# imjaegyun/super_resolution

Measured on AMD Instinct MI355X. Metric: SR output megapixels/sec, HAT-S x4, 1280x720 LR in, higher is better.
Workload: dtype bf16; 1 GPU; HAT-S x4, one 3x720x1280 LR frame per GPU, full-frame forward; upscale=4, parallelism=dp1

## Files before the change

super_resolution_amd/csrc/hat_mlp.hip:

```cpp
#include <type_traits>

#include "hat_common.h"

namespace {

struct LdsBases { unsigned b0, b1, b2; };
constexpr unsigned LB_STEP = 61440;
__device__ __forceinline__ LdsBases lds_bases(const char* lane_base) {
    typedef __attribute__((address_space(3))) char lds_char;
    LdsBases r;
    r.b0 = (unsigned)(uintptr_t)(lds_char*)lane_base;
    r.b1 = r.b0 + LB_STEP;
    r.b2 = r.b0 + 2 * LB_STEP;
    asm volatile("" : "+v"(r.b0), "+v"(r.b1), "+v"(r.b2));
    return r;
}
template <typename V> __device__ __forceinline__ V lds_at(const LdsBases& lb, unsigned off) {
    const unsigned base = off < LB_STEP ? lb.b0 : (off < 2 * LB_STEP ? lb.b1 : lb.b2);
    const unsigned rel = off < LB_STEP ? off : (off < 2 * LB_STEP ? off - LB_STEP : off - 2 * LB_STEP);
    return *(__attribute__((address_space(3))) const V*)(uintptr_t)(base + rel);
}

constexpr int ML_C = 144, ML_HID = 288, ML_NT1 = ML_HID / 16, ML_NT2 = ML_C / 16, ML_KK = ML_HID / 32;
constexpr int ML_W1F = ML_NT1 * 4 * 1024;
constexpr int ML_W1H = ML_NT1 * 512;
constexpr int ML_NREG = 4;
constexpr int ML_W2F = (ML_NT2 * ML_KK - ML_NREG) * 1024;
constexpr int ML_OFF_W1H = ML_W1F, ML_OFF_W2 = ML_W1F + ML_W1H, ML_OFF_B1 = ML_OFF_W2 + ML_W2F, ML_OFF_B2 = ML_OFF_B1 + ML_HID * 4;
constexpr int ML_LDS = ML_OFF_B2 + ML_C * 4;
constexpr int ML_WAVES = 8, ML_NTHR = ML_WAVES * 64;

template <bool OUTF32, bool R16 = false>
__global__ __launch_bounds__(ML_NTHR) void ocab_mlp_kernel(const HatMlpDesc d, long npix, long tiles) {
    using M = MT<bf16_t>;
    typedef bf16_t T;
    typedef M::frag_t frag_t;
    extern __shared__ __attribute__((aligned(16))) char smem[];
    const int tid = threadIdx.x, lane = tid & 63, g = lane >> 4, c16 = lane & 15;
    const int wave = tid >> 6;
    {
        const char* w1 = reinterpret_cast<const char*>(d.w1f);
        for (int i = tid; i < (ML_W1F + ML_W1H) / 16; i += ML_NTHR)
            *reinterpret_cast<u32x4*>(smem + (size_t)i * 16) = *reinterpret_cast<const u32x4*>(w1 + (size_t)i * 16);
        const char* w2 = reinterpret_cast<const char*>(d.w2f);
        for (int i = tid; i < ML_W2F / 16; i += ML_NTHR)
            *reinterpret_cast<u32x4*>(smem + ML_OFF_W2 + (size_t)i * 16) = *reinterpret_cast<const u32x4*>(w2 + (size_t)i * 16);
        float* b1 = reinterpret_cast<float*>(smem + ML_OFF_B1);
        for (int i = tid; i < ML_HID; i += ML_NTHR) b1[i] = d.b1[i];
        float* b2 = reinterpret_cast<float*>(smem + ML_OFF_B2);
        for (int i = tid; i < ML_C; i += ML_NTHR) b2[i] = d.b2[i];
    }
    frag_t w2r[ML_NREG];
#pragma unroll
    for (int i = 0; i < ML_NREG; ++i)
        w2r[i] = M::load(reinterpret_cast<const T*>(d.w2f) + (size_t)(ML_NT2 * ML_KK - ML_NREG + i) * 512 + lane * 8);
    __syncthreads();

    const T* xg = reinterpret_cast<const T*>(d.x);
    const float* b1l = reinterpret_cast<const float*>(smem + ML_OFF_B1);
    const float* b2l = reinterpret_cast<const float*>(smem + ML_OFF_B2);
    typedef short s16x4 __attribute__((ext_vector_type(4)));
    struct XB { frag_t f[4]; s16x4 h; };
    auto load_x = [&](long tile, XB& xb) {
        long p = tile * 16 + c16;
        p = p < npix ? p : npix - 1;
        const T* row = xg + p * d.ldx;
#pragma unroll
        for (int ks = 0; ks < 4; ++ks) xb.f[ks] = M::load(row + ks * 32 + 8 * g);
        xb.h = *reinterpret_cast<const s16x4*>(row + 128 + 4 * g);
    };
    using r1_t = std::conditional_t<R16, h4raw, f32x4>;
    auto load_r = [&](long tile, r1_t (&r)[ML_NT2]) {
        long p = tile * 16 + c16;
        p = p < npix ? p : npix - 1;
#pragma unroll
        for (int nt = 0; nt < ML_NT2; ++nt) {
            if constexpr (R16) r[nt] = load_h4raw(reinterpret_cast<const _Float16*>(d.r1) + p * d.ldr1 + nt * 16 + 4 * g);
            else r[nt] = *reinterpret_cast<const f32x4*>(d.r1 + p * d.ldr1 + nt * 16 + 4 * g);
        }
    };

    const long stride = (long)gridDim.x * ML_WAVES;
    long tile = (long)blockIdx.x * ML_WAVES + wave;
    XB xcur, xnxt;
    r1_t r1v[ML_NT2];
    load_x(tile, xcur);
    load_x(tile + stride, xnxt);
    load_r(tile, r1v);
    for (; tile < tiles; tile += stride) {
        const long p = tile * 16 + c16;
        const long pc = p < npix ? p : npix - 1;
        int wofs = lane * 16;
        asm volatile("" : "+v"(wofs));
        const char* wl = smem + wofs;
        const char* wl8 = smem + ML_OFF_W1H + (wofs >> 1);
        const LdsBases lb = lds_bases(wl), lb8 = lds_bases(smem + (wofs >> 1));
        frag_t pf[ML_KK];
        {
            struct W1 { s16x4 h; f32x4 b; frag_t f[4]; };
            W1 ws[2];
            auto rd1 = [&](int nt, W1& w) {
                w.h = lds_at<s16x4>(lb8, ML_OFF_W1H + nt * 512);
                w.b = *reinterpret_cast<const f32x4*>(b1l + nt * 16 + 4 * g);
#pragma unroll
                for (int ks = 0; ks < 4; ++ks) w.f[ks] = lds_at<frag_t>(lb, (nt * 4 + ks) * 1024);
            };
            rd1(0, ws[0]);
            f32x4 a[2];
#pragma unroll
            for (int nt = 0; nt < ML_NT1; ++nt) {
                if (nt + 1 < ML_NT1) rd1(nt + 1, ws[(nt + 1) & 1]);
                const W1& w = ws[nt & 1];
                const f32x4 tail = __builtin_amdgcn_mfma_f32_16x16x16bf16_1k(w.h, xcur.h, w.b, 0, 0, 0);
                f32x4 ai = f32x4{0.f, 0.f, 0.f, 0.f};
#pragma unroll
                for (int ks = 0; ks < 4; ++ks) ai = M::mma(w.f[ks], xcur.f[ks], ai);
                a[nt & 1] = ai + tail;
                if (nt & 1) {
#pragma unroll
                    for (int j = 0; j < 4; ++j) {
                        pf[nt >> 1][j] = (bf16_t)gelu_act<T>(a[0][j]);
                        pf[nt >> 1][4 + j] = (bf16_t)gelu_act<T>(a[1][j]);
                    }
                }
                __builtin_amdgcn_sched_barrier(0);
            }
        }
        f32x4 acc[ML_NT2];
        {
            constexpr int NF = ML_NT2 * ML_KK - ML_NREG, AD = 3;
            frag_t ring[AD + 1];
            auto rd2 = [&](int f) { ring[f % (AD + 1)] = lds_at<frag_t>(lb, ML_OFF_W2 + f * 1024); };
#pragma unroll
            for (int f = 0; f < AD; ++f) rd2(f);
#pragma unroll
            for (int nt = 0; nt < ML_NT2; ++nt) {
                if constexpr (R16) acc[nt] = *reinterpret_cast<const f32x4*>(b2l + nt * 16 + 4 * g) + h4raw_to_f32(r1v[nt]);
                else acc[nt] = *reinterpret_cast<const f32x4*>(b2l + nt * 16 + 4 * g) + r1v[nt];
#pragma unroll
                for (int kk = 0; kk < ML_KK; ++kk) {
                    const int f = nt * ML_KK + kk;
                    if (f + AD < NF) rd2(f + AD);
                    if (f < NF)
                        acc[nt] = M::mma(ring[f % (AD + 1)], pf[kk], acc[nt]);
                    else
                        acc[nt] = M::mma(w2r[f - NF], pf[kk], acc[nt]);
                    __builtin_amdgcn_sched_barrier(0);
                }
            }
        }
        xcur = xnxt;
        if constexpr (OUTF32) {
            float* o = reinterpret_cast<float*>(d.out) + pc * d.ldo;
#pragma unroll
            for (int nt = 0; nt < ML_NT2; ++nt) *reinterpret_cast<f32x4*>(o + nt * 16 + 4 * g) = acc[nt];
        } else {
            bf16_t* o = reinterpret_cast<bf16_t*>(d.out) + pc * d.ldo;
#pragma unroll
            for (int nt = 0; nt + 1 < ML_NT2; nt += 2) store_pair_bf16(o, nt * 16, g, acc[nt], acc[nt + 1]);
            Vec4<T>::store(o + (ML_NT2 - 1) * 16 + 4 * g, acc[ML_NT2 - 1]);
        }
        load_x(tile + 2 * stride, xnxt);
        load_r(tile + stride, r1v);
    }
}

constexpr int QK_NT = 27, QK_N = QK_NT * 16;
constexpr int QK_WF = QK_NT * 4 * 1024, QK_WH = QK_NT * 512, QK_OFF_B = QK_WF + QK_WH, QK_LDS = QK_OFF_B + QK_N * 4;

__global__ __launch_bounds__(ML_NTHR) void ocab_qkv_kernel(const HatMlpDesc d, long npix, long tiles) {
    using M = MT<bf16_t>;
    typedef bf16_t T;
    typedef M::frag_t frag_t;
    typedef short s16x4 __attribute__((ext_vector_type(4)));
    extern __shared__ __attribute__((aligned(16))) char smem[];
    const int tid = threadIdx.x, lane = tid & 63, g = lane >> 4, c16 = lane & 15;
    const int wave = tid >> 6;
    {
        const char* w1 = reinterpret_cast<const char*>(d.w1f);
        for (int i = tid; i < (QK_WF + QK_WH) / 16; i += ML_NTHR)
            *reinterpret_cast<u32x4*>(smem + (size_t)i * 16) = *reinterpret_cast<const u32x4*>(w1 + (size_t)i * 16);
        float* bl = reinterpret_cast<float*>(smem + QK_OFF_B);
        for (int i = tid; i < QK_N; i += ML_NTHR) bl[i] = d.b1[i];
    }
    __syncthreads();
    const T* xg = reinterpret_cast<const T*>(d.x);
    const float* bl = reinterpret_cast<const float*>(smem + QK_OFF_B);
    struct XB { frag_t f[4]; s16x4 h; };
    auto load_x = [&](long tile, XB& xb) {
        long p = tile * 16 + c16;
        p = p < npix ? p : npix - 1;
        const T* row = xg + p * d.ldx;
#pragma unroll
        for (int ks = 0; ks < 4; ++ks) xb.f[ks] = M::load(row + ks * 32 + 8 * g);
        xb.h = *reinterpret_cast<const s16x4*>(row + 128 + 4 * g);
    };
// ... 31 lines not shown
#pragma unroll
            for (int ks = 0; ks < 4; ++ks) ai = M::mma(w.f[ks], xcur.f[ks], ai);
            a[nt & 1] = ai + tail;
            if (nt & 1) store_pair_bf16(o, (nt - 1) * 16, g, a[0], a[1]);
            else if (nt == QK_NT - 1) last = a[0];
            __builtin_amdgcn_sched_barrier(0);
        }
        Vec4<T>::store(o + (QK_NT - 1) * 16 + 4 * g, last);
        xcur = xnxt;
        load_x(tile + 2 * stride, xnxt);
    }
}

}

extern "C" int hat_ocab_qkv(const HatMlpDesc* dp, void* stream) {
    if (!dp) return HAT_EINVAL;
    const HatMlpDesc& d = *dp;
    if (!d.x || !d.w1f || !d.b1 || !d.out || d.B < 1 || d.H < 1 || d.W < 1) return HAT_EINVAL;
    if (d.C != ML_C || d.hidden != QK_N || d.dtype != HAT_BF16) return HAT_EUNSUPPORTED;
    if (d.ldx < ML_C || d.ldx % 8 || d.ldo < QK_N || d.ldo % 8 || reinterpret_cast<uintptr_t>(d.out) % 16) return HAT_EINVAL;
    const long npix = (long)d.B * d.H * d.W, tiles = (npix + 15) / 16;
    int gx = 256;
    if ((long)gx * ML_WAVES > tiles) gx = (int)((tiles + ML_WAVES - 1) / ML_WAVES);
    hipError_t e = hipFuncSetAttribute(reinterpret_cast<const void*>(ocab_qkv_kernel), hipFuncAttributeMaxDynamicSharedMemorySize, QK_LDS);
    if (e != hipSuccess) return (int)e;
    HAT_LAUNCH(ocab_qkv_kernel, dim3(gx), dim3(ML_NTHR), QK_LDS, reinterpret_cast<hipStream_t>(stream), d, npix, tiles);
    return hat_check_launch();
}

extern "C" int hat_ocab_mlp(const HatMlpDesc* dp, void* stream) {
    if (!dp) return HAT_EINVAL;
    const HatMlpDesc& d = *dp;
    if (!d.x || !d.w1f || !d.b1 || !d.w2f || !d.b2 || !d.r1 || !d.out) return HAT_EINVAL;
    if (d.B < 1 || d.H < 1 || d.W < 1) return HAT_EINVAL;
    if (d.C != ML_C || d.hidden != ML_HID || d.dtype != HAT_BF16) return HAT_EUNSUPPORTED;
    if (d.ldx < ML_C || d.ldx % 8 || d.ldr1 < ML_C || d.ldr1 % 4 || d.ldo < ML_C) return HAT_EINVAL;
    if ((d.out_f32 & ~3) != 0 || d.out_f32 == 3) return HAT_EINVAL;
    const bool out_f32 = (d.out_f32 & 1) != 0, r16 = (d.out_f32 & 2) != 0;
    if (r16 && reinterpret_cast<uintptr_t>(d.r1) % 8) return HAT_EINVAL;
    if (out_f32 ? d.ldo % 4 : (d.ldo % 8 || reinterpret_cast<uintptr_t>(d.out) % 16)) return HAT_EINVAL;
    const long npix = (long)d.B * d.H * d.W, tiles = (npix + 15) / 16;
    int gx = 256;
    if ((long)gx * ML_WAVES > tiles) gx = (int)((tiles + ML_WAVES - 1) / ML_WAVES);
    hipStream_t s = reinterpret_cast<hipStream_t>(stream);
    void (*kern)(const HatMlpDesc, long, long) = out_f32 ? ocab_mlp_kernel<true> : r16 ? ocab_mlp_kernel<false, true> : ocab_mlp_kernel<false>;
    hipError_t e = hipFuncSetAttribute(reinterpret_cast<const void*>(kern), hipFuncAttributeMaxDynamicSharedMemorySize, ML_LDS);
    if (e != hipSuccess) return (int)e;
    HAT_LAUNCH(kern, dim3(gx), dim3(ML_NTHR), ML_LDS, s, d, npix, tiles);
    return hat_check_launch();
}
```

super_resolution_amd/engine.py:

```python
from __future__ import annotations

import contextlib
import dataclasses
import math
import os
import warnings
from typing import Dict, Optional

import torch

from . import ops
from .engine_base import EngineBase
from .frame_boundary import FrameBoundary
from .ops import (ACT_GELU, ACT_LRELU, ACT_NONE, O_NCHW_F32, O_NHWC_F32, O_NHWC_T, O_PIXSHUF_T, X_NCHW_F32_MEAN, X_NHWC_F32, X_NHWC_T)
from .packing import _ESC

RGB_MEAN = (0.4488, 0.4371, 0.4040)


def _r8(x: int) -> int:
    return (x + 7) // 8 * 8


def _r4(x: int) -> int:
# ... 36 lines not shown
        return cls(t16_guard=(get("t16_guard") or "defer"), **kw)


class _T16Guard:

    def __init__(self, dev):
        self.slot = torch.zeros(1, dtype=torch.int32, device=dev)
        self.host = torch.zeros(1, dtype=torch.int32).pin_memory()
        self.event = torch.cuda.Event()
        self.pending = 0

    def word(self) -> int:
        return int(self.host[0]) & 0xFFFFFFFF


class _Packed:

    def __getitem__(self, key):
        try:
            return getattr(self, key)
        except AttributeError:
            raise KeyError(key) from None


class _Hab(_Packed):
    fold = ffn = ffn3 = fc1 = fc2 = bias256 = None
    tail = "aggr"
    next_ln = None
    out16 = False


class _Ocab(_Packed):
    qkvf = mlpf = esc = fh0 = fh2 = None


class _Naf(_Packed):

    def __init__(self, c, head, blocks, tail):
        self.c, self.head, self.blocks, self.tail = c, head, blocks, tail


class _Group(_Packed):
    to_conv = ocab16 = out16 = False
    conv_ln = None

    def __init__(self, heads, habs, ocab, conv):
        self.heads, self.habs, self.ocab, self.conv = heads, habs, ocab, conv


class _Fwd:

    def __init__(self, eng, w, B, H, W, band, one_stream):
        self.B, self.H, self.W, self.N = B, H, W, H * W
        self.C, self.dt, self.ldc = eng.C, eng.dtype, _r8(eng.C)
        self.geo = dict(B=B, H=H, W=W, dtype=eng.dtype)
        self.w, self.band, self.one_stream = w, band, one_stream
        self.t = self.gin = w["tA"]
        self.have_n = self.have_n16 = False
        self.nblk = ops.layernorm_blocks()

    def ln(self, src, dst, gb, out_f32=False, gap_c=0):
        ops.layernorm(src, dst, gb[0], gb[1], B=self.B, npix=self.N, C_=self.C, ldy=(self.C if out_f32 else self.ldc),
                      out_f32=out_f32, dtype=self.dt, gap=(self.w["gap"] if gap_c else None), gap_c=gap_c)

    def pooled(self, src, ld, C_, dst, off=0, r0=None, r1=None, c0=0, c1=None):
        bd, w = self.band, self.w
# ... 162 lines not shown
            hb.ffn3 = ops.pack_ffn3(*fw, *hb.n2, dev)
        if (hb.fold is None and C == 180 and fp16_ok and ops.tail3_supported(C, hid2 // 2, dt) and hb.esc.pdim == 16
                and hb.esc.aggr.frag and not opt.no_hab_tail):
            f3 = ops.pack_ffn3(*fw, *hb.n2, dev)
            if ops.hab_tail_supported(f3, hb.esc.aggr, w2raw.shape[1], dt):
                hb.ffn3, hb.tail180_ok = f3, True
                hb.bias256 = torch.zeros(256, **f32)
                hb.bias256[:C] = vec(hb.esc.aggr_keys[1])
        return hb

    def _pack_ocab(self, sd, p, heads):
        cfg, dt, dev, C = self.cfg, self.dtype, self.dev, self.C
        vec = lambda k: sd[k].detach().to(dtype=torch.float32, device=dev).contiguous()
        ws, wse = self.ws, self.wse
        M = ws + wse - 1
        shift = (ws - wse + 1 - (ws - 1)) * (M + 1)
        rot = (torch.arange(M * M) + shift) % (M * M)
        d = C // heads
        qscale = cfg.get("qk_scale") or d ** -0.5
        qlog2 = (ops.ocab_attention_log2_supported(C, heads, ws, wse, dt) and not (self.focus or self.topk < 1.0)
                 and not self.opt.no_attn_log2 and d % 2 == 0 and _r8(C) == C)
        if qlog2:
            qscale = qscale * ops.LOG2E
        table = sd[p + ".relative_position_bias_table"].detach().to(torch.float32).cpu()
        oc = _Ocab()
        oc.n1 = (vec(p + ".norm1.weight"), vec(p + ".norm1.bias"))
        oc.n2 = (vec(p + ".norm2.weight"), vec(p + ".norm2.bias"))
        oc.q = self._lin(sd, p + ".q_proj.weight", p + ".q_proj.bias", scale=qscale)
        oc.kv = self._lin(sd, p + ".kv_proj.weight", p + ".kv_proj.bias")
        oc.proj = self._lin(sd, p + ".proj.weight", p + ".proj.bias")
        oc.mlp0 = self._lin(sd, p + ".mlp.0.weight", p + ".mlp.0.bias")
        oc.mlp2 = self._lin(sd, p + ".mlp.2.weight", p + ".mlp.2.bias")
        if ops.ocab_mlp_supported(C, sd[p + ".mlp.0.weight"].shape[0], dt) and _r8(C) == C and not self.opt.no_ocab_mlp:
            oc.mlpf = ops.pack_ocab_mlp(sd[p + ".mlp.0.weight"], sd[p + ".mlp.0.bias"], sd[p + ".mlp.2.weight"], sd[p + ".mlp.2.bias"], dev)
        oc.bias_rot = table[rot].t().contiguous().to(dev)
        oc.qlog2 = qlog2
        if C == 144 and dt == ops.HAT_BF16 and not cfg.get("ocab_esc_enable", False) and not self.opt.no_ocab_qkv:
            oc.qkvf = ops.pack_ocab_qkv(sd[p + ".q_proj.weight"], sd.get(p + ".q_proj.bias"), sd[p + ".kv_proj.weight"],
                                        sd.get(p + ".kv_proj.bias"), qscale, dev)
        if cfg.get("ocab_esc_enable", False):
            oc.esc = self._esc(sd, p + ".esc_core", p + ".esc_plk", cfg["ocab_esc_pdim"], cfg["ocab_esc_kernel"])
        if self.focus:
            oc.fh0 = ops.pack_conv_weight(sd[p + ".focus_head.0.weight"], sd[p + ".focus_head.0.bias"], dt, dev)
            oc.fh2 = ops.pack_conv_weight(sd[p + ".focus_head.2.weight"], sd[p + ".focus_head.2.bias"], dt, dev)
        return oc

    def _pack_ps(self, sd, key, r):
        w = sd[key + ".weight"]
        o = w.shape[0]
        cps = o // (r * r)
        n = torch.arange(o)
        perm = (n % cps) * (r * r) + n // cps
        return ops.pack_conv_weight(w, sd[key + ".bias"], self.dtype, self.dev, out_perm=perm)

    def _resolve(self):
        layers, dt, C = self.layers, self.dtype, self.C
        escs = [hb.esc for G in layers for hb in G.habs] + [G.ocab.esc for G in layers if G.ocab.esc is not None]
        wide = any(e.npad > 16 for e in escs)
        for gi, G in enumerate(layers):
            oc = G.ocab
            for i, hb in enumerate(G.habs):
                nh = G.habs[i + 1] if i + 1 < len(G.habs) else None
                hb.next_ln = (nh.n1, nh.esc.pdim) if nh is not None else (oc.n1, oc.esc.pdim if oc.esc is not None else 0)
                if hb.fold is not None:
                    hb.tail = "fused144" if hb.tail144_ok and not wide else "aggr_cab"
                else:
                    hb.tail = "fused180" if hb.tail180_ok and hb.next_ln[1] <= 16 else "aggr"
            G.to_conv = bool(G.conv is not None and dt == ops.HAT_BF16 and _r8(C) == C and oc.mlp2.frag and not self.opt.no_bf16_conv_in)
            cv = G.conv
            if cv is not None and dt == ops.HAT_BF16 and not self.opt.no_conv_ln and cv.n_slices == 1 and cv.nout == cv.nt * 16:
                if gi + 1 < len(layers):
                    nhs = layers[gi + 1].habs
                    nxt, gap_c = (nhs[0].n1, nhs[0].esc.pdim) if nhs else (None, 0)
                else:
                    nxt, gap_c = (self.norm, 0) if self.conv_after_body is not None else (None, 0)
                G.conv_ln = (nxt, gap_c) if nxt is not None and gap_c in (0, 4, 8, 12, 16) else None
        self._plan_t16()
        self.u8_fused = self.conv_last_sweep is not None and self.conv_last_sweep[2] == 3
        hab0 = layers[0].habs[0] if layers and layers[0].habs else None
        self._hab0 = hab0
        self._yw = max([16] + [e.npad for e in escs])
        self._kpad = max([hab0.esc.kpad if hab0 else 0] + [G.ocab.esc.kpad for G in layers if G.ocab.esc is not None])

    def _plan_t16(self):
        layers = self.layers
        for G in layers:
            G.ocab16 = G.out16 = False
            for hb in G.habs:
                hb.out16 = False
        if not self.t16:
            return
        tail16 = lambda hb: hb.tail == "fused144" and hb.ffn3.C == 144
        conv16 = lambda G: bool(G.conv is not None and not G.conv.frag and G.conv.ksize > 1 and G.conv.nt == 9
                                and G.conv.n_slices == 1 and G.conv.nout == 144)
        for G in layers:
            oc = G.ocab
            G.ocab16 = bool(G.habs and tail16(G.habs[-1]) and G.to_conv and oc.mlpf is not None and oc.proj.frag
                            and oc.proj.nt == 9 and getattr(oc.proj, "ksplit", None) is None and oc.esc is None)
            for i, hb in enumerate(G.habs):
                hb.out16 = tail16(hb) and (G.ocab16 if i + 1 == len(G.habs) else tail16(G.habs[i + 1]))
# ... 466 lines not shown
        w, oc, esc, bd, t, C, ldc, geo = f.w, G.ocab, G.ocab.esc, f.band, f.t, self.C, f.ldc, f.geo
        nblk = f.nblk
        if bd is not None:
            yield ("halo", [((w["n"] if f.have_n else t), self._ocab_halo(oc))])
        if not f.have_n:
            f.ln(t, w["n"], oc.n1, gap_c=(esc.pdim if esc else 0))
            nblk = ops.layernorm_blocks()
        kv_src = w["n"]
        if esc is not None:
            if bd is not None:
                gl, gg = f.gstat(esc)
                f.pooled(w["n"], ldc, esc.pdim, gl)
                yield ("reduce", [(gl, gg, esc.pdim)])
                self._esc_w(esc, w, f.B, bd.Hfull, f.W, 1, gap=gg)
                self._esc_conv(esc, w, w["n"], f.B, f.H, f.W)
            else:
                self._esc_lk(esc, w, w["n"], f.B, f.H, f.W, nblk)
            self._run_lin(esc.aggr, w["n"], w["yesc"], **geo, ldx=ldc, ldo=ldc, x0=w["y16"], c_split=esc.pdim, ldx0=w["y16"].shape[2])
            kv_src = w["yesc"]
        if oc.qkvf is not None:
            ops.ocab_qkv(oc.qkvf, w["n"], w["qkv"], **geo, ldx=ldc, ldo=432)
            qbuf, kvbuf, ldq, ldkv = w["qkv"], w["qkv"].view(-1)[144:], 432, 432
        else:
            qbuf, kvbuf, ldq, ldkv = w["q"], w["kv"], ldc, w["kv"].shape[2]
            s0 = torch.cuda.current_stream(self.dev)
            s1 = self._side_stream(f)
            s1.wait_stream(s0)
            with torch.cuda.stream(s1):
                self._run_lin(oc.q, w["n"], w["q"], **geo, ldx=ldc, ldo=ldc)
            self._run_lin(oc.kv, kv_src, w["kv"], **geo, ldx=ldc, ldo=w["kv"].shape[2])
            s0.wait_stream(s1)
        self._ocab_attention(f, G, kv_src, qbuf, kvbuf, ldq, ldkv)
        tout = w["tB"] if t is w["tA"] else t
        if oc.proj.frag:
            self._run_lin(oc.proj, w["ao"], tout, **geo, ldx=ldc, ldo=C, out_mode=O_NHWC_F32, r1=t, ldr1=C,
                          ln=oc.n2, ln_out=w["n"], ld_ln=ldc, **({"sat": self._sat(True)} if tout.dtype == torch.float16 and self._armed else {}))
        else:
            self._run_lin(oc.proj, w["ao"], tout, **geo, ldx=ldc, ldo=C, out_mode=O_NHWC_F32, r1=t, ldr1=C)
            f.ln(tout, w["n"], oc.n2)
        if oc.mlpf is not None:
            dst = w["ao"] if as_conv_input else tout
            ops.ocab_mlp(oc.mlpf, w["n"], tout, dst, B=f.B, H=f.H, W=f.W, ldx=ldc, ldr1=C, ldo=(ldc if as_conv_input else C),
                         out_f32=not as_conv_input, dtype=f.dt)
            return dst
        self._run_lin(oc.mlp0, w["n"], w["g"], **geo, ldx=ldc, ldo=w["g"].shape[2], act=ACT_GELU)
        if as_conv_input:
            self._run_lin(oc.mlp2, w["g"], w["ao"], **geo, ldx=w["g"].shape[2], ldo=ldc, out_mode=O_NHWC_T, r1=tout, ldr1=C)
            return w["ao"]
        self._run_lin(oc.mlp2, w["g"], tout, **geo, ldx=w["g"].shape[2], ldo=C, out_mode=O_NHWC_F32, r1=tout, ldr1=C)
        return tout

    def _ocab_attention(self, f: _Fwd, G: _Group, kv_src, qbuf, kvbuf, ldq, ldkv):
        w, oc, C, ldc, ws, wse = f.w, G.ocab, self.C, f.ldc, self.ws, self.wse
        if not (self.focus or self.topk < 1.0):
            ops.ocab_attention(qbuf, kvbuf, oc.bias_rot, w["ao"], B=f.B, H=f.H, W=f.W, C_=C, heads=G.heads, ws=ws, wse=wse,
                               ldq=ldq, ldkv=ldkv, ldo=ldc, dtype=f.dt, q_log2=oc.qlog2)
            return
        nk, pad = wse * wse, (wse - ws + 1) // 2
        if self.focus:
            ops.conv(oc.fh0, kv_src, w["fh"], **f.geo, ldx=ldc, ldo=w["fh"].shape[2], act=ACT_GELU, n_store=_r4(C // 4))
            ops.conv(oc.fh2, w["fh"], w["sal"], **f.geo, ldx=w["fh"].shape[2], ldo=8, n_store=4, out_mode=O_NHWC_F32)
        k_keep = max(1, int(self.topk * nk)) if self.topk < 1.0 else nk
        ops.ocab_keybias(w["sal"] if self.focus else None, kvbuf, w["kb"], B=f.B, H=f.H, W=f.W, C_=C, ws=ws, wse=wse, pad=pad,
                         k_keep=k_keep, ldsal=(-8 if f.dt == ops.HAT_BF16 else 8), ldkv=ldkv, dtype=f.dt)
        ops.ocab_attention_kb(qbuf, kvbuf, oc.bias_rot, w["kb"], w["ao"], B=f.B, H=f.H, W=f.W, C_=C, heads=G.heads, ws=ws,
                              wse=wse, pad=pad, ldq=ldq, ldkv=ldkv, ldo=ldc, dtype=f.dt)

    def _group_end(self, f: _Fwd, G: _Group, tout):
        w, tA, C = f.w, f.w["tA"], self.C
# ... 74 lines not shown
```

super_resolution_amd/ops.py:

```python
from __future__ import annotations

import collections
import ctypes as C
from typing import Optional

import numpy as np
import torch

from . import _lib
from ._lib import (ACT_GELU, ACT_LRELU, ACT_LRELU02, ACT_NONE, HAT_BF16, HAT_F32, O_FOLD2_NCHW_F32, O_NCHW_F32, O_NHWC_F32, O_NHWC_T, O_PIXSHUF_T,
                   X_NCHW_F32_MEAN, X_NHWC_F32, X_NHWC_T, HatAggrCabDesc, HatCabFoldDesc, HatConvDesc, HatFfnDesc, HatHabTailDesc, HatMlpDesc, HatNafFoldDesc,
                   HatNafHalfDesc, HatEscConvFfnDesc)
from .packing import (ESC_HID_PAD, FP16_SAFE, KC, NAF_WIDTHS, TORCH_DTYPE, PackedConv, PackedEscFfn, PackedFFN, PackedMlp, PackedNafBlock, choose_nt,
                      esc_geo_ensemble, pack_esc_convffn, PackedEscRealSkip, ESCFP_HID_PAD, PackedEscFpLk, bicubic_phase_table, escfp_rank1_fold,
                      pack_escfp_convffn, pack_escfp_lk, dysample_fold, pack_escreal_skip, pack_nearest_conv,
                      LTE_HIDDEN, PackedLte, pack_lte,
                      UNI_UPSAMPLERS, PackedEscRealMSkip, conv_nearest_fold, pack_conv_nearest, pack_escrealm_skip, pack_pixshuf_conv, pixshuf_perm,
                      choose_nt_linear, naf_ffn_fold, naf_frags, pack_naf_block,
                      ffn_fp16_range_bound, pack_upfold, pack_cab_squeeze, pack_cab_w2f, pack_conv_weight, pack_ffn, pack_ffn2, pack_ffn3,
                      pack_linear_weight, pack_ocab_mlp, pack_ocab_qkv, pack_pointwise)

DTYPE_CODE = {"f32": HAT_F32, "fp32": HAT_F32, "float32": HAT_F32, "bf16": HAT_BF16, "bfloat16": HAT_BF16}


# ... 175 lines not shown
    _timed(f"dwgate_kernel<{_TNAME[dtype]}>", 2.0 * 9 * 2 * hid * B * H * W, lambda: _lib.check(
        lib.hat_dwconv_gate(_ptr(u), _ptr(wdw), _ptr(bdw), _ptr(out), B, H, W, hid, ldu, ldo, dtype, _stream()),
        "hat_dwconv_gate"))


def ocab_keybias(sal, kv, kb, *, B: int, H: int, W: int, C_: int, ws: int, wse: int, pad: int, k_keep: int, ldsal: int, ldkv: int,
                 dtype: int):
    lib = _lib.load()
    _timed("keybias_kernel", 0.0, lambda: _lib.check(
        lib.hat_ocab_keybias(_ptr(sal), ldsal, _ptr(kv), ldkv, _ptr(kb), B, H, W, C_, ws, wse, pad, k_keep, dtype, _stream()), "hat_ocab_keybias"))


def ocab_attention_kb(q, kv, bias_rot, kb, out, *, B: int, H: int, W: int, C_: int, heads: int, ws: int, wse: int, pad: int, ldq: int,
                      ldkv: int, ldo: int, dtype: int):
    lib = _lib.load()
    _timed(f"ocab_attn_kernel<{_TNAME[dtype]}, kb>", 2.0 * 2 * wse * wse * C_ * B * H * W, lambda: _lib.check(
        lib.hat_ocab_attention_kb(_ptr(q), _ptr(kv), _ptr(bias_rot), _ptr(kb), _ptr(out), B, H, W, C_, heads, ws, wse, pad, ldq, ldkv, ldo,
                                  dtype, _stream()), "hat_ocab_attention_kb"))


def ocab_mlp_supported(C_: int, hidden: int, dtype: int) -> bool:
    return C_ == 144 and hidden == 288 and dtype == HAT_BF16


def ocab_qkv(pm: PackedMlp, x, out, *, B: int, H: int, W: int, ldx: int, ldo: int, dtype: int):
    lib = _lib.load()
    d = HatMlpDesc()
    d.x, d.w1f, d.b1, d.out = _ptr(x), _ptr(pm.w1f), _ptr(pm.b1), _ptr(out)
    d.B, d.H, d.W, d.C, d.hidden, d.ldx, d.ldo, d.dtype = B, H, W, pm.C, pm.hidden, ldx, ldo, dtype
    _timed("ocab_qkv_kernel", 2.0 * pm.C * pm.hidden * B * H * W, lambda: _lib.check(lib.hat_ocab_qkv(C.byref(d), _stream()), "hat_ocab_qkv"),
           tag=f"qkv {pm.C}->{pm.hidden} {H}x{W}", nbytes=float(B * H * W) * 2 * (ldx + pm.hidden))


def ocab_mlp(pm: PackedMlp, x, r1, out, *, B: int, H: int, W: int, ldx: int, ldr1: int, ldo: int, out_f32: bool, dtype: int):
    lib = _lib.load()
    d = HatMlpDesc()
    d.x, d.w1f, d.b1, d.w2f, d.b2, d.r1, d.out = _ptr(x), _ptr(pm.w1f), _ptr(pm.b1), _ptr(pm.w2f), _ptr(pm.b2), _ptr(r1), _ptr(out)
    r16 = r1.dtype == torch.float16
    d.B, d.H, d.W, d.C, d.hidden, d.ldx, d.ldr1, d.ldo, d.dtype = B, H, W, pm.C, pm.hidden, ldx, ldr1, ldo, dtype
    d.out_f32 = int(out_f32) | (2 if r16 else 0)
    _timed(f"ocab_mlp_kernel<{'true' if out_f32 else 'false'}>", 2.0 * 2 * pm.C * pm.hidden * B * H * W,
           lambda: _lib.check(lib.hat_ocab_mlp(C.byref(d), _stream()), "hat_ocab_mlp"),
           tag=f"mlp {pm.C}->{pm.hidden}->{pm.C} {H}x{W}",
           nbytes=float(B * H * W) * (2 * ldx + (2 if r16 else 4) * pm.C + (4 if out_f32 else 2) * pm.C))


def sgfn_gate(u, wdw, bdw, out, *, B: int, H: int, W: int, half: int, ldu: int, ldo: int, dtype: int):
    lib = _lib.load()
    _timed(f"sgfn_gate_kernel<{_TNAME[dtype]}>", 2.0 * 9 * half * B * H * W, lambda: _lib.check(
        lib.hat_sgfn_gate(_ptr(u), _ptr(wdw), _ptr(bdw), _ptr(out), B, H, W, half, ldu, ldo, dtype, _stream()), "hat_sgfn_gate"))


def naf_tiles(H: int, W: int) -> int:
    n = _lib.load().hat_naf_half_tiles(H, W)
    _lib.check(min(n, 0), "hat_naf_half_tiles")
    return n


def naf_half(r_in, g_out, w1, b1, dww, dwb, *, B: int, H: int, W: int, C_: int, dtype: int, ldr: Optional[int] = None, ldo: Optional[int] = None,
             gprev=None, ldg: Optional[int] = None, wf=None, wf_bstride: int = 0, bf=None, bf_bstride: int = 0, r_out=None, partials=None):
    lib = _lib.load()
    d = HatNafHalfDesc()
    d.r_in, d.gprev, d.wf, d.bf, d.r_out = _ptr(r_in), _ptr(gprev), _ptr(wf), _ptr(bf), _ptr(r_out)
    d.w1, d.b1, d.dww, d.dwb, d.g_out, d.partials = _ptr(w1), _ptr(b1), _ptr(dww), _ptr(dwb), _ptr(g_out), _ptr(partials)
    d.wf_bstride, d.bf_bstride = wf_bstride, bf_bstride
    d.B, d.H, d.W, d.C, d.dtype = B, H, W, C_, dtype
    d.ldr, d.ldg, d.ldo = (C_ if ldr is None else ldr), (C_ if ldg is None else ldg), (C_ if ldo is None else ldo)
    form = "a" if gprev is None else ("b" if w1 is not None else "proj")
    es, npx = (2 if dtype == HAT_BF16 else 4), float(B * H * W)
    flops = 2.0 * npx * C_ * ((2 * C_ if w1 is not None else 0) + (C_ if gprev is not None else 0)) + (2.0 * 9 * 2 * C_ * npx if w1 is not None else 0.0)
    nbytes = npx * C_ * (4 + (4 + es if gprev is not None else 0) + (es if w1 is not None else 0))
    _timed(f"naf_half_kernel<{_TNAME[dtype]}, {C_}>", flops, lambda: _lib.check(lib.hat_naf_half(C.byref(d), _stream()), f"hat_naf_half(c={C_}, form {form})"),
           tag=f"naf {form} c{C_} {H}x{W}{' pool' if partials is not None else ''}", nbytes=nbytes)


def naf_fold(partials, blk: PackedNafBlock, wf, bf, *, B: int, H: int, W: int, C_: int, dtype: int):
    lib = _lib.load()
# ... 1079 lines not shown
    what = "hat_hab_tail3" if sat is None else "hat_hab_tail3_guarded"
    if pf.C == 180:
        flops = B * H * W * (2.0 * pf.C * pf.C + 2.0 * pf.C * 2 * pf.hid + 2.0 * 9 * 2 * pf.hid + 2.0 * pf.hid * pf.C)
        nbytes = B * H * W * (2.0 * ldn_in + 32 + 2.0 * ldr2 + 4.0 * pf.C + 4.0 * pf.C + (2 * ldn if ln1 is not None else 0))
        _timed("tail3l_kernel", flops, lambda: _lib.check(tail3(), what), nbytes=nbytes)
        return
    flops = B * H * W * (2.0 * pf.C * (pf.C + 72) + 2.0 * pf.C * 2 * pf.hid + 2.0 * 9 * 2 * pf.hid + 2.0 * pf.hid * pf.C)
    nbytes = B * H * W * (2.0 * ldn_in + 32 + 16 + (2.0 if in_half else 4.0) * pf.C + (2.0 if out_half else 4.0) * pf.C + (2 * ldn if ln1 is not None else 0))
    if pf.layout == "tail3":
        _timed("tail3_kernel", flops, lambda: _lib.check(tail3(), what), nbytes=nbytes)
        return
    _timed("ffn2_kernel<aggr>", flops, lambda: _lib.check(lib.hat_hab_tail(C.byref(h), _stream()), "hat_hab_tail"), nbytes=nbytes)


_PW_SHAPES = {(9, 5), (18, 5), (9, 9), (12, 6), (23, 6), (12, 12), (4, 1), (4, 2)}


def linear_supported(nout: int, cin: int, dtype: int) -> bool:
    nt, _ = choose_nt_linear(nout, cin, dtype)
    ks = -(-cin // 32)
    lds = nt * ks * 64 * 8 * (2 if dtype == HAT_BF16 else 4)
    return (nt, ks) in _PW_SHAPES and lds <= 163840 and cin % 4 == 0


def linear(pw: PackedConv, x: torch.Tensor, out: torch.Tensor, *, B: int, H: int, W: int, dtype: int, ldx: int, ldo: int,
           out_mode: int = O_NHWC_T, act: int = ACT_NONE, n_store: Optional[int] = None, x0: Optional[torch.Tensor] = None,
           c_split: int = 0, ldx0: int = 0, r1: Optional[torch.Tensor] = None, ldr1: int = 0, r2: Optional[torch.Tensor] = None,
           ldr2: int = 0, r2scale: Optional[torch.Tensor] = None, r2scale_bstride: int = 0, ln=None,
           ln_out: Optional[torch.Tensor] = None, ld_ln: int = 0, ln_ones: bool = False, sat: Optional[torch.Tensor] = None):
    lib = _lib.load()
    d = HatConvDesc()
    d.x, d.x0, d.w, d.bias, d.out = _ptr(x), _ptr(x0), _ptr(pw.w), _ptr(pw.bias), _ptr(out)
    d.r1, d.r2, d.r2scale = _ptr(r1), _ptr(r2), _ptr(r2scale)
    if ln is not None:
        d.ln_g, d.ln_b, d.ln_out, d.ld_ln, d.ln_ones = _ptr(ln[0]), _ptr(ln[1]), _ptr(ln_out), ld_ln, int(ln_ones)
    d.B, d.H, d.W, d.Cin, d.ldx, d.x_mode = B, H, W, pw.cin, ldx, X_NHWC_T
    d.c_split, d.ldx0, d.ksize, d.Kpad, d.nt, d.n_slices = c_split, ldx0, 1, pw.kpad, pw.nt, pw.n_slices
    d.n_store = pw.nout if n_store is None else n_store
    d.ldo, d.out_mode, d.act, d.ldr1, d.ldr2, d.r2scale_bstride, d.dtype = ldo, out_mode, act, ldr1, ldr2, r2scale_bstride, dtype
    d.reserved0 = _stream16(r1, out, out_mode)
    flops = 2.0 * B * H * W * pw.cin * pw.nout
    _timed(f"pw_kernel<{_TNAME[dtype]}, {pw.nt}, {pw.kpad // 32}>", flops,
           lambda: _lib.check(lib.hat_linear(C.byref(d), _stream()) if sat is None else lib.hat_linear_guarded(C.byref(d), _sat_ptr(sat), _stream()),
                              f"hat_linear{'' if sat is None else '_guarded'}(Cin={pw.cin}, N={pw.nout})"),
           tag=f"lin {pw.cin}->{pw.nout} {H}x{W} o{out_mode}{' r1' if r1 is not None else ''}{' r2' if r2 is not None else ''}")


_T3_SHAPES = {(1, 144), (9, 8), (1, 24), (4, 8)}


def conv3x3_small_supported(nout: int, cin: int, dtype: int = HAT_BF16) -> bool:
    nt, n_slices = choose_nt(nout)
    cin_p = (cin + 7) // 8 * 8
    lds = nt * (-(-9 * cin_p // 32)) * 64 * 8 * (2 if dtype == HAT_BF16 else 4)
    return (nt, cin_p) in _T3_SHAPES and n_slices == 1 and lds <= 81920


def _c3_desc(pw, B, H, W, dtype, ldx):
    d = HatConvDesc()
    d.B, d.H, d.W, d.Cin, d.ldx, d.x_mode = B, H, W, pw.cin, ldx, X_NHWC_T
    d.ksize, d.Kpad, d.nt, d.n_slices, d.dtype = 3, pw.kpad, pw.nt, 1, dtype
    return d


def conv3x3_small_groups(pw: PackedConv, B: int, H: int, W: int, dtype: int) -> int:
    lib = _lib.load()
    d = _c3_desc(pw, B, H, W, dtype, 8)
# ... 49 lines not shown
```

super_resolution_amd/packing.py:

```python
from __future__ import annotations

from typing import Optional

import torch

from ._lib import HAT_BF16, HAT_F32

TORCH_DTYPE = {HAT_F32: torch.float32, HAT_BF16: torch.bfloat16}
KC = {HAT_F32: 32, HAT_BF16: 64}


class PackedConv:
    __slots__ = ("w", "bias", "ksize", "cin", "kpad", "nt", "n_slices", "nout", "w_bstride", "frag", "ksplit")

    def __init__(self, w, bias, ksize, cin, kpad, nt, n_slices, nout, w_bstride=0, frag=False):
        self.w, self.bias, self.ksize, self.cin, self.kpad = w, bias, ksize, cin, kpad
        self.nt, self.n_slices, self.nout, self.w_bstride = nt, n_slices, nout, w_bstride
        self.frag = frag
        self.ksplit = None

    @property
    def npad(self):
        return self.nt * 16 * self.n_slices


class PackedMlp:
    __slots__ = ("w1f", "b1", "w2f", "b2", "C", "hidden")


class PackedFFN:
    __slots__ = ("w1f", "b1", "dww", "dwb", "w2f", "b2", "chunks", "C", "hid", "nt", "ks", "layout")


def choose_nt(nout: int):
    best = None
    for nt in (12, 9, 8, 4, 1):
        npad = -(-nout // (16 * nt)) * 16 * nt
        cost = npad * (nt + 2) / nt
        if best is None or cost < best[0]:
            best = (cost, nt, npad // (16 * nt))
    return best[1], best[2]


def choose_nt_linear(nout: int, cin: int, dtype: int):
    if nout == 288 and -(-cin // 32) == 5 and dtype == HAT_BF16:
        return 18, 1
    if nout == 360 and -(-cin // 32) == 6 and dtype == HAT_BF16:
        return 23, 1
    return choose_nt(nout)


def _f32(t: torch.Tensor) -> torch.Tensor:
    return t.detach().to(torch.float32).cpu()


def _pad(m: torch.Tensor, rows: int, cols: Optional[int] = None) -> torch.Tensor:
    if m.dim() == 1:
        out = torch.zeros(rows)
        out[:m.shape[0]] = m
    else:
# ... 38 lines not shown
    kpad = -(-w.shape[1] // kc) * kc
    npad = nt * 16 * n_slices
    return PackedConv(_pad(w, npad, kpad).to(TORCH_DTYPE[dtype]).to(device).contiguous(), _pad(b, npad).to(device), kh, i, kpad, nt, n_slices, o)


def pack_linear_weight(weight: torch.Tensor, bias: Optional[torch.Tensor], dtype: int, device, scale: float = 1.0) -> PackedConv:
    w = _f32(weight)
    ksize, cin = 1, None
    if w.dim() == 4 and w.shape[-1] > 1:
        cin, ksize = w.shape[1], w.shape[2]
        w = _tap_major(w)
    w = w.reshape(w.shape[0], -1) * scale
    o, i = w.shape
    b = (torch.zeros(o) if bias is None else _f32(bias)) * scale
    nt, n_slices = choose_nt_linear(o, i, dtype) if ksize == 1 else choose_nt(o)
    ks = -(-i // 32)
    npad = nt * 16 * n_slices
    wf = frags(_pad(w, npad, ks * 32)).reshape(n_slices, nt, ks, 64, 8)
    return PackedConv(wf.to(TORCH_DTYPE[dtype]).contiguous().to(device), _pad(b, npad).to(device), ksize, (i if cin is None else cin),
                      ks * 32, nt, n_slices, o, frag=True)


def pack_pointwise(weight: torch.Tensor, bias: Optional[torch.Tensor], dtype: int, device, scale: float = 1.0) -> PackedConv:
    from .ops import linear_supported
    if linear_supported(weight.shape[0], weight.shape[1], dtype):
        return pack_linear_weight(weight, bias, dtype, device, scale=scale)
    return pack_conv_weight(weight, bias, dtype, device, scale=scale)


def _pack_fc1_frags(W1: torch.Tensor) -> torch.Tensor:
    return torch.cat([frags(W1[:, :128]).reshape(-1), frags(W1[:, 128:], jn=4).reshape(-1)])


def pack_ocab_mlp(fc1_w, fc1_b, fc2_w, fc2_b, device) -> PackedMlp:
    W1, b1, W2, b2 = _f32(fc1_w), _f32(fc1_b), _f32(fc2_w), _f32(fc2_b)
    hid, C_ = W1.shape
    assert (C_, hid) == (144, 288) and W2.shape == (C_, hid)
    p = PackedMlp()
    p.w1f = _pack_fc1_frags(W1).to(torch.bfloat16).contiguous().to(device)
    p.w2f = frags(W2, "acc").to(torch.bfloat16).contiguous().to(device)
    p.b1, p.b2, p.C, p.hidden = b1.contiguous().to(device), b2.contiguous().to(device), C_, hid
    return p


def pack_ocab_qkv(q_w, q_b, kv_w, kv_b, qscale: float, device) -> PackedMlp:
    Wq, Wkv = _f32(q_w) * qscale, _f32(kv_w)
    bq = (torch.zeros(Wq.shape[0]) if q_b is None else _f32(q_b)) * qscale
    bkv = torch.zeros(Wkv.shape[0]) if kv_b is None else _f32(kv_b)
    W = torch.cat([Wq, Wkv], 0)
    assert W.shape == (432, 144)
    p = PackedMlp()
    p.w1f = _pack_fc1_frags(W).to(torch.bfloat16).contiguous().to(device)
    p.b1 = torch.cat([bq, bkv]).contiguous().to(device)
    p.w2f = p.b2 = None
    p.C, p.hidden = 144, 432
    return p


def pack_cab_squeeze(weight: torch.Tensor, bias: torch.Tensor, device):
    w = _f32(weight)
    mid, cin = w.shape[0], w.shape[1]
    A = torch.zeros(6, 16, 32 * -(-cin // 32))
    for kx in range(3):
        A[2 * kx, 0:mid, :cin] = w[:, :, 0, kx]
        A[2 * kx, 8:8 + mid, :cin] = w[:, :, 1, kx]
        A[2 * kx + 1, 0:mid, :cin] = w[:, :, 2, kx]
    return frags(A.reshape(96, -1)).to(torch.bfloat16).contiguous().to(device), _pad(_f32(bias), 8).to(device)


def pack_cab_w2f(w2: torch.Tensor, device) -> torch.Tensor:
    w = _f32(w2)
    C_, mid = w.shape[0], w.shape[1]
    full = torch.zeros(-(-C_ // 16) * 16, 12, 8)
    full[:C_, :9, :mid] = w.reshape(C_, mid, 9).permute(0, 2, 1)
    return frags(full.reshape(-1, 96)).contiguous().to(device)


FP16_SAFE = 6.0e4


def ffn_fp16_range_bound(fc1_w, fc1_b, dw_w, dw_b, ln_g, ln_b) -> float:
    f = lambda t: t.detach().to(torch.float64).cpu()
    W1, b1, Wd, bd, g_, b_ = f(fc1_w), f(fc1_b), f(dw_w).reshape(-1, 9), f(dw_b), f(ln_g), f(ln_b)
    C_ = W1.shape[1]
    hid = W1.shape[0] // 2
    U = (C_ ** 0.5) * (W1 * g_[None, :]).norm(dim=1) + (W1 @ b_ + b1).abs()
    A = Wd.abs().sum(1) * U + bd.abs()
# ... 419 lines not shown
```

Before: 359.4 MP/s.

## Fuse OCAB LayerNorm2 into MLP kernel by normalizing residual in-register

Adds an LN template path to the OCAB MLP kernel that computes LayerNorm2 from the fp32/fp16 residual it already loads, with lane reductions via permlane swaps, and builds the bf16 input fragments in registers. The LN gamma and beta are folded into fc1 weights and bias at pack time, so the proj kernel no longer writes a normalized bf16 tensor and the MLP no longer reads one. This saves one write and one read of the activation per block, at the cost of extra ALU work and register pressure inside the MLP kernel. It also changes rounding, since normalization now happens in-kernel on folded weights.

```diff
diff --git a/super_resolution_amd/csrc/hat_mlp.hip b/super_resolution_amd/csrc/hat_mlp.hip
--- a/super_resolution_amd/csrc/hat_mlp.hip
+++ b/super_resolution_amd/csrc/hat_mlp.hip
@@ -30,7 +30,7 @@
 constexpr int ML_LDS = ML_OFF_B2 + ML_C * 4;
 constexpr int ML_WAVES = 8, ML_NTHR = ML_WAVES * 64;
 
-template <bool OUTF32, bool R16 = false>
+template <bool OUTF32, bool R16 = false, bool LN = false>
 __global__ __launch_bounds__(ML_NTHR) void ocab_mlp_kernel(const HatMlpDesc d, long npix, long tiles) {
     using M = MT<bf16_t>;
     typedef bf16_t T;
@@ -80,16 +80,67 @@
         }
     };
 
+    auto r_f32 = [&](const r1_t& r) {
+        if constexpr (R16) return h4raw_to_f32(r);
+        else return r;
+    };
+
     const long stride = (long)gridDim.x * ML_WAVES;
     long tile = (long)blockIdx.x * ML_WAVES + wave;
     XB xcur, xnxt;
     r1_t r1v[ML_NT2];
-    load_x(tile, xcur);
-    load_x(tile + stride, xnxt);
-    load_r(tile, r1v);
+    r1_t rnxt[LN ? ML_NT2 : 1];
+    if constexpr (LN) {
+        load_r(tile, r1v);
+        load_r(tile + stride, rnxt);
+    } else {
+        load_x(tile, xcur);
+        load_x(tile + stride, xnxt);
+        load_r(tile, r1v);
+    }
     for (; tile < tiles; tile += stride) {
         const long p = tile * 16 + c16;
         const long pc = p < npix ? p : npix - 1;
+        if constexpr (LN) {
+            typedef float f32x2 __attribute__((ext_vector_type(2)));
+            auto sum4 = [](float s) {
+                const unsigned u = __builtin_bit_cast(unsigned, s);
+                const auto a = __builtin_amdgcn_permlane16_swap(u, u, false, false);
+                const float t = __builtin_bit_cast(float, (unsigned)a[0]) + __builtin_bit_cast(float, (unsigned)a[1]);
+                const unsigned w = __builtin_bit_cast(unsigned, t);
+                const auto b = __builtin_amdgcn_permlane32_swap(w, w, false, false);
+                return __builtin_bit_cast(float, (unsigned)b[0]) + __builtin_bit_cast(float, (unsigned)b[1]);
+            };
+            f32x4 v[ML_NT2];
+            f32x2 s2 = {0.f, 0.f};
+#pragma unroll
+            for (int nt = 0; nt < ML_NT2; ++nt) {
+                v[nt] = r_f32(r1v[nt]);
+                s2 += f32x2{v[nt][0], v[nt][1]} + f32x2{v[nt][2], v[nt][3]};
+            }
+            const float mean = sum4(s2[0] + s2[1]) * (1.0f / (float)ML_C);
+            f32x2 q2 = {0.f, 0.f};
+#pragma unroll
+            for (int nt = 0; nt < ML_NT2; ++nt) {
+                const f32x4 dl = v[nt] - mean;
+                q2 += f32x2{dl[0], dl[1]} * f32x2{dl[0], dl[1]} + f32x2{dl[2], dl[3]} * f32x2{dl[2], dl[3]};
+            }
+            const float rstd = __builtin_amdgcn_rsqf(sum4(q2[0] + q2[1]) * (1.0f / (float)ML_C) + 1e-5f);
+            const float nmr = -mean * rstd;
+#pragma unroll
+            for (int ks = 0; ks < 4; ++ks) {
+                const f32x4 n0 = v[2 * ks] * rstd + nmr, n1 = v[2 * ks + 1] * rstd + nmr;
+#pragma unroll
+                for (int j = 0; j < 4; ++j) {
+                    xcur.f[ks][j] = (bf16_t)n0[j];
+                    xcur.f[ks][4 + j] = (bf16_t)n1[j];
+                }
+            }
+            const f32x4 n8 = v[ML_NT2 - 1] * rstd + nmr;
+            typedef bf16_t v4b __attribute__((ext_vector_type(4)));
+            const v4b hb = {(bf16_t)n8[0], (bf16_t)n8[1], (bf16_t)n8[2], (bf16_t)n8[3]};
+            xcur.h = __builtin_bit_cast(s16x4, hb);
+        }
         int wofs = lane * 16;
         asm volatile("" : "+v"(wofs));
         const char* wl = smem + wofs;
@@ -135,8 +186,7 @@
             for (int f = 0; f < AD; ++f) rd2(f);
 #pragma unroll
             for (int nt = 0; nt < ML_NT2; ++nt) {
-                if constexpr (R16) acc[nt] = *reinterpret_cast<const f32x4*>(b2l + nt * 16 + 4 * g) + h4raw_to_f32(r1v[nt]);
-                else acc[nt] = *reinterpret_cast<const f32x4*>(b2l + nt * 16 + 4 * g) + r1v[nt];
+                acc[nt] = *reinterpret_cast<const f32x4*>(b2l + nt * 16 + 4 * g) + r_f32(r1v[nt]);
 #pragma unroll
                 for (int kk = 0; kk < ML_KK; ++kk) {
                     const int f = nt * ML_KK + kk;
@@ -149,7 +199,7 @@
                 }
             }
         }
-        xcur = xnxt;
+        if constexpr (!LN) xcur = xnxt;
         if constexpr (OUTF32) {
             float* o = reinterpret_cast<float*>(d.out) + pc * d.ldo;
 #pragma unroll
@@ -160,8 +210,14 @@
             for (int nt = 0; nt + 1 < ML_NT2; nt += 2) store_pair_bf16(o, nt * 16, g, acc[nt], acc[nt + 1]);
             Vec4<T>::store(o + (ML_NT2 - 1) * 16 + 4 * g, acc[ML_NT2 - 1]);
         }
-        load_x(tile + 2 * stride, xnxt);
-        load_r(tile + stride, r1v);
+        if constexpr (LN) {
+#pragma unroll
+            for (int nt = 0; nt < ML_NT2; ++nt) r1v[nt] = rnxt[nt];
+            load_r(tile + 2 * stride, rnxt);
+        } else {
+            load_x(tile + 2 * stride, xnxt);
+            load_r(tile + stride, r1v);
+        }
     }
 }
 
@@ -259,12 +315,13 @@
 extern "C" int hat_ocab_mlp(const HatMlpDesc* dp, void* stream) {
     if (!dp) return HAT_EINVAL;
     const HatMlpDesc& d = *dp;
-    if (!d.x || !d.w1f || !d.b1 || !d.w2f || !d.b2 || !d.r1 || !d.out) return HAT_EINVAL;
+    if (!d.w1f || !d.b1 || !d.w2f || !d.b2 || !d.r1 || !d.out) return HAT_EINVAL;
     if (d.B < 1 || d.H < 1 || d.W < 1) return HAT_EINVAL;
     if (d.C != ML_C || d.hidden != ML_HID || d.dtype != HAT_BF16) return HAT_EUNSUPPORTED;
-    if (d.ldx < ML_C || d.ldx % 8 || d.ldr1 < ML_C || d.ldr1 % 4 || d.ldo < ML_C) return HAT_EINVAL;
-    if ((d.out_f32 & ~3) != 0 || d.out_f32 == 3) return HAT_EINVAL;
-    const bool out_f32 = (d.out_f32 & 1) != 0, r16 = (d.out_f32 & 2) != 0;
+    if ((d.out_f32 & ~7) != 0 || (d.out_f32 & 3) == 3) return HAT_EINVAL;
+    const bool out_f32 = (d.out_f32 & 1) != 0, r16 = (d.out_f32 & 2) != 0, ln = (d.out_f32 & 4) != 0;
+    if (!ln && (!d.x || d.ldx < ML_C || d.ldx % 8)) return HAT_EINVAL;
+    if (d.ldr1 < ML_C || d.ldr1 % 4 || d.ldo < ML_C) return HAT_EINVAL;
     if (r16 && reinterpret_cast<uintptr_t>(d.r1) % 8) return HAT_EINVAL;
     if (out_f32 ? d.ldo % 4 : (d.ldo % 8 || reinterpret_cast<uintptr_t>(d.out) % 16)) return HAT_EINVAL;
     const long npix = (long)d.B * d.H * d.W, tiles = (npix + 15) / 16;
@@ -272,6 +329,7 @@
     if ((long)gx * ML_WAVES > tiles) gx = (int)((tiles + ML_WAVES - 1) / ML_WAVES);
     hipStream_t s = reinterpret_cast<hipStream_t>(stream);
     void (*kern)(const HatMlpDesc, long, long) = out_f32 ? ocab_mlp_kernel<true> : r16 ? ocab_mlp_kernel<false, true> : ocab_mlp_kernel<false>;
+    if (ln) kern = out_f32 ? ocab_mlp_kernel<true, false, true> : r16 ? ocab_mlp_kernel<false, true, true> : ocab_mlp_kernel<false, false, true>;
     hipError_t e = hipFuncSetAttribute(reinterpret_cast<const void*>(kern), hipFuncAttributeMaxDynamicSharedMemorySize, ML_LDS);
     if (e != hipSuccess) return (int)e;
     HAT_LAUNCH(kern, dim3(gx), dim3(ML_NTHR), ML_LDS, s, d, npix, tiles);
diff --git a/super_resolution_amd/engine.py b/super_resolution_amd/engine.py
--- a/super_resolution_amd/engine.py
+++ b/super_resolution_amd/engine.py
@@ -92,6 +92,7 @@
 
 class _Ocab(_Packed):
     qkvf = mlpf = esc = fh0 = fh2 = None
+    mlp_ln = False
 
 
 class _Naf(_Packed):
@@ -320,7 +321,8 @@
         oc.mlp0 = self._lin(sd, p + ".mlp.0.weight", p + ".mlp.0.bias")
         oc.mlp2 = self._lin(sd, p + ".mlp.2.weight", p + ".mlp.2.bias")
         if ops.ocab_mlp_supported(C, sd[p + ".mlp.0.weight"].shape[0], dt) and _r8(C) == C and not self.opt.no_ocab_mlp:
-            oc.mlpf = ops.pack_ocab_mlp(sd[p + ".mlp.0.weight"], sd[p + ".mlp.0.bias"], sd[p + ".mlp.2.weight"], sd[p + ".mlp.2.bias"], dev)
+            oc.mlpf = ops.pack_ocab_mlp(sd[p + ".mlp.0.weight"], sd[p + ".mlp.0.bias"], sd[p + ".mlp.2.weight"], sd[p + ".mlp.2.bias"], dev,
+                                        ln_g=sd[p + ".norm2.weight"], ln_b=sd[p + ".norm2.bias"])
         oc.bias_rot = table[rot].t().contiguous().to(dev)
         oc.qlog2 = qlog2
         if C == 144 and dt == ops.HAT_BF16 and not cfg.get("ocab_esc_enable", False) and not self.opt.no_ocab_qkv:
@@ -354,6 +356,8 @@
                     hb.tail = "fused144" if hb.tail144_ok and not wide else "aggr_cab"
                 else:
                     hb.tail = "fused180" if hb.tail180_ok and hb.next_ln[1] <= 16 else "aggr"
+            oc.mlp_ln = bool(oc.mlpf is not None and oc.mlpf.w1n is not None and oc.proj.frag
+                             and getattr(oc.proj, "ksplit", None) is None and oc.esc is None)
             G.to_conv = bool(G.conv is not None and dt == ops.HAT_BF16 and _r8(C) == C and oc.mlp2.frag and not self.opt.no_bf16_conv_in)
             cv = G.conv
             if cv is not None and dt == ops.HAT_BF16 and not self.opt.no_conv_ln and cv.n_slices == 1 and cv.nout == cv.nt * 16:
@@ -886,9 +890,16 @@
             s0.wait_stream(s1)
         self._ocab_attention(f, G, kv_src, qbuf, kvbuf, ldq, ldkv)
         tout = w["tB"] if t is w["tA"] else t
+        sat = {"sat": self._sat(True)} if tout.dtype == torch.float16 and self._armed else {}
+        if oc.mlp_ln:
+            self._run_lin(oc.proj, w["ao"], tout, **geo, ldx=ldc, ldo=C, out_mode=O_NHWC_F32, r1=t, ldr1=C, ln=oc.n2, ln_out=None, **sat)
+            dst = w["ao"] if as_conv_input else tout
+            ops.ocab_mlp(oc.mlpf, None, tout, dst, B=f.B, H=f.H, W=f.W, ldx=0, ldr1=C, ldo=(ldc if as_conv_input else C),
+                         out_f32=not as_conv_input, dtype=f.dt, ln_from_r1=True)
+            return dst
         if oc.proj.frag:
             self._run_lin(oc.proj, w["ao"], tout, **geo, ldx=ldc, ldo=C, out_mode=O_NHWC_F32, r1=t, ldr1=C,
-                          ln=oc.n2, ln_out=w["n"], ld_ln=ldc, **({"sat": self._sat(True)} if tout.dtype == torch.float16 and self._armed else {}))
+                          ln=oc.n2, ln_out=w["n"], ld_ln=ldc, **sat)
         else:
             self._run_lin(oc.proj, w["ao"], tout, **geo, ldx=ldc, ldo=C, out_mode=O_NHWC_F32, r1=t, ldr1=C)
             f.ln(tout, w["n"], oc.n2)
diff --git a/super_resolution_amd/ops.py b/super_resolution_amd/ops.py
--- a/super_resolution_amd/ops.py
+++ b/super_resolution_amd/ops.py
@@ -231,17 +231,25 @@
            tag=f"qkv {pm.C}->{pm.hidden} {H}x{W}", nbytes=float(B * H * W) * 2 * (ldx + pm.hidden))
 
 
-def ocab_mlp(pm: PackedMlp, x, r1, out, *, B: int, H: int, W: int, ldx: int, ldr1: int, ldo: int, out_f32: bool, dtype: int):
+def ocab_mlp(pm: PackedMlp, x, r1, out, *, B: int, H: int, W: int, ldx: int, ldr1: int, ldo: int, out_f32: bool, dtype: int,
+             ln_from_r1: bool = False):
+    if ln_from_r1 and pm.w1n is None:
+        raise ValueError("ln_from_r1 needs a PackedMlp packed with LayerNorm2's gamma and beta (pack_ocab_mlp(..., ln_g, ln_b))")
     lib = _lib.load()
     d = HatMlpDesc()
-    d.x, d.w1f, d.b1, d.w2f, d.b2, d.r1, d.out = _ptr(x), _ptr(pm.w1f), _ptr(pm.b1), _ptr(pm.w2f), _ptr(pm.b2), _ptr(r1), _ptr(out)
+    w1f, b1 = (pm.w1n, pm.b1n) if ln_from_r1 else (pm.w1f, pm.b1)
+    d.x, d.w1f, d.b1, d.w2f, d.b2, d.r1, d.out = (None if ln_from_r1 else _ptr(x)), _ptr(w1f), _ptr(b1), _ptr(pm.w2f), _ptr(pm.b2), _ptr(r1), _ptr(out)
     r16 = r1.dtype == torch.float16
-    d.B, d.H, d.W, d.C, d.hidden, d.ldx, d.ldr1, d.ldo, d.dtype = B, H, W, pm.C, pm.hidden, ldx, ldr1, ldo, dtype
-    d.out_f32 = int(out_f32) | (2 if r16 else 0)
-    _timed(f"ocab_mlp_kernel<{'true' if out_f32 else 'false'}>", 2.0 * 2 * pm.C * pm.hidden * B * H * W,
+    d.B, d.H, d.W, d.C, d.hidden, d.ldx, d.ldr1, d.ldo, d.dtype = B, H, W, pm.C, pm.hidden, (0 if ln_from_r1 else ldx), ldr1, ldo, dtype
+    d.out_f32 = int(out_f32) | (2 if r16 else 0) | (4 if ln_from_r1 else 0)
+    _timed(f"ocab_mlp_kernel<{'true' if out_f32 else 'false'}{', ln' if ln_from_r1 else ''}>", 2.0 * 2 * pm.C * pm.hidden * B * H * W,
            lambda: _lib.check(lib.hat_ocab_mlp(C.byref(d), _stream()), "hat_ocab_mlp"),
-           tag=f"mlp {pm.C}->{pm.hidden}->{pm.C} {H}x{W}",
-           nbytes=float(B * H * W) * (2 * ldx + (2 if r16 else 4) * pm.C + (4 if out_f32 else 2) * pm.C))
+           tag=f"mlp {'ln ' if ln_from_r1 else ''}{pm.C}->{pm.hidden}->{pm.C} {H}x{W}",
+           nbytes=float(B * H * W) * ((0 if ln_from_r1 else 2 * ldx) + (2 if r16 else 4) * pm.C + (4 if out_f32 else 2) * pm.C))
+
+
+def ocab_mlp_ln(pm: PackedMlp, r1, out, *, B: int, H: int, W: int, ldr1: int, ldo: int, out_f32: bool, dtype: int):
+    ocab_mlp(pm, None, r1, out, B=B, H=H, W=W, ldx=0, ldr1=ldr1, ldo=ldo, out_f32=out_f32, dtype=dtype, ln_from_r1=True)
 
 
 def sgfn_gate(u, wdw, bdw, out, *, B: int, H: int, W: int, half: int, ldu: int, ldo: int, dtype: int):
@@ -1387,7 +1395,7 @@
     d = HatConvDesc()
     d.x, d.x0, d.w, d.bias, d.out = _ptr(x), _ptr(x0), _ptr(pw.w), _ptr(pw.bias), _ptr(out)
     d.r1, d.r2, d.r2scale = _ptr(r1), _ptr(r2), _ptr(r2scale)
-    if ln is not None:
+    if ln is not None and ln_out is not None:
         d.ln_g, d.ln_b, d.ln_out, d.ld_ln, d.ln_ones = _ptr(ln[0]), _ptr(ln[1]), _ptr(ln_out), ld_ln, int(ln_ones)
     d.B, d.H, d.W, d.Cin, d.ldx, d.x_mode = B, H, W, pw.cin, ldx, X_NHWC_T
     d.c_split, d.ldx0, d.ksize, d.Kpad, d.nt, d.n_slices = c_split, ldx0, 1, pw.kpad, pw.nt, pw.n_slices
diff --git a/super_resolution_amd/packing.py b/super_resolution_amd/packing.py
--- a/super_resolution_amd/packing.py
+++ b/super_resolution_amd/packing.py
@@ -25,7 +25,7 @@
 
 
 class PackedMlp:
-    __slots__ = ("w1f", "b1", "w2f", "b2", "C", "hidden")
+    __slots__ = ("w1f", "b1", "w2f", "b2", "C", "hidden", "w1n", "b1n")
 
 
 class PackedFFN:
@@ -130,11 +130,24 @@
     return torch.cat([frags(W1[:, :128]).reshape(-1), frags(W1[:, 128:], jn=4).reshape(-1)])
 
 
-def pack_ocab_mlp(fc1_w, fc1_b, fc2_w, fc2_b, device) -> PackedMlp:
+def _pack_fc1_frags_acc(W1: torch.Tensor) -> torch.Tensor:
+    return torch.cat([frags(W1[:, :128], "acc").reshape(-1), frags(W1[:, 128:], jn=4).reshape(-1)])
+
+
+def ocab_mlp_ln_fold(W1, b1, ln_g, ln_b):
+    return W1 * ln_g[None, :], b1 + W1 @ ln_b
+
+
+def pack_ocab_mlp(fc1_w, fc1_b, fc2_w, fc2_b, device, ln_g=None, ln_b=None) -> PackedMlp:
     W1, b1, W2, b2 = _f32(fc1_w), _f32(fc1_b), _f32(fc2_w), _f32(fc2_b)
     hid, C_ = W1.shape
     assert (C_, hid) == (144, 288) and W2.shape == (C_, hid)
     p = PackedMlp()
+    p.w1n = p.b1n = None
+    if ln_g is not None:
+        W1n, b1n = ocab_mlp_ln_fold(W1, b1, _f32(ln_g), _f32(ln_b))
+        p.w1n = _pack_fc1_frags_acc(W1n).to(torch.bfloat16).contiguous().to(device)
+        p.b1n = b1n.contiguous().to(device)
     p.w1f = _pack_fc1_frags(W1).to(torch.bfloat16).contiguous().to(device)
     p.w2f = frags(W2, "acc").to(torch.bfloat16).contiguous().to(device)
     p.b1, p.b2, p.C, p.hidden = b1.contiguous().to(device), b2.contiguous().to(device), C_, hid
@@ -150,7 +163,7 @@
     p = PackedMlp()
     p.w1f = _pack_fc1_frags(W).to(torch.bfloat16).contiguous().to(device)
     p.b1 = torch.cat([bq, bkv]).contiguous().to(device)
-    p.w2f = p.b2 = None
+    p.w2f = p.b2 = p.w1n = p.b1n = None
     p.C, p.hidden = 144, 432
     return p
 
```

New measurement: 361.6 MP/s, median of 6. No clear change (+0.6%).
